# Kunvuthi/cobalt_smart_lender_ai

Hardware: AMD Instinct MI355X
Metric: rows/sec GBDT train on 10M-row LendingClub-shaped tabular; AUC parity (higher is better)
Workload: dtype fp32; 1 GPU; global_batch=10000000, rows_per_gpu=10000000, parallelism=dp1, n_features=20, trees=300, max_depth=7

## Files before the change

### cobalt_smart_lender_ai_amd/_native.py

```python
from __future__ import annotations

import ctypes
import os
import threading
from pathlib import Path

import torch

from . import build as _build
from .config import knob

_lock = threading.Lock()
_lib: ctypes.CDLL | None = None
_err: str | None = None

c_void_p = ctypes.c_void_p
c_int = ctypes.c_int
c_int64 = ctypes.c_int64
c_double = ctypes.c_double
c_float = ctypes.c_float
c_char_p = ctypes.c_char_p


class NativeUnavailable(RuntimeError):
    pass


_SIGS: dict[str, tuple] = {
    "cobalt_gbdt_create": (c_int, [c_void_p, ctypes.POINTER(c_void_p)]),
    "cobalt_heap_to_trees": (ctypes.c_int64, [c_void_p, c_int, c_int] + [c_void_p] * 10),
    "cobalt_gbdt_set_data": (c_int, [c_void_p] * 9),
    "cobalt_gbdt_grow": (c_int, [c_void_p, c_int, c_int, c_void_p]),
    "cobalt_gbdt_fetch_trees": (c_int, [c_void_p, c_int, c_int, c_void_p, c_void_p]),
    "cobalt_gbdt_max_nodes": (c_int, [c_void_p]),
    "cobalt_gbdt_set_start": (c_int, [c_void_p, c_int]),
    "cobalt_gbdt_set_binary_labels": (c_int, [c_void_p, c_float, c_void_p]),
    "cobalt_gbdt_set_monotone": (c_int, [c_void_p, c_void_p, c_int]),
    "cobalt_gbdt_set_interaction": (c_int, [c_void_p, c_void_p, c_int, c_int]),
    "cobalt_gbdt_destroy": (c_int, [c_void_p]),
    "cobalt_gbdt_reuse": (c_int, [c_void_p, c_void_p]),
    "cobalt_gbdt_grow_sampled": (c_int, [c_void_p, c_int, c_void_p]),
    "cobalt_gbdt_set_rows": (c_int, [c_void_p, c_int64]),
    "cobalt_gbdt_error": (c_int, [c_void_p]),
    "cobalt_gbdt_ox_init": (c_int, [c_void_p, c_int64, c_void_p, c_void_p, c_void_p]),
    "cobalt_gbdt_ox_begin": (c_int, [c_void_p, c_int, c_void_p]),
    "cobalt_gbdt_ox_page": (c_int, [c_void_p, c_void_p, c_int, c_int64, c_int64, c_int, c_int, c_void_p]),
    "cobalt_gbdt_ox_level": (c_int, [c_void_p, c_int, c_int, c_void_p]),
    "cobalt_gbdt_ox_end": (c_int, [c_void_p, c_int, c_void_p]),
    "cobalt_gbdt_set_fault": (c_int, [c_void_p, c_int]),
    "cobalt_gbdt_tree_ptr": (c_void_p, [c_void_p, c_int]),
    "cobalt_ooc_page": (c_int, [c_void_p, c_int, c_int64, c_int64, c_int, c_void_p, c_int, c_void_p, c_void_p, c_void_p,
                                ctypes.c_uint64, c_int64, ctypes.c_double, ctypes.c_double, ctypes.c_double,
                                c_void_p, c_void_p, c_int64, c_void_p, c_void_p, c_void_p]),
    "cobalt_ooc_bins": (c_int, []),
    "cobalt_gbdt_plan": (c_int, [c_void_p, c_void_p]),
# ... 118 lines not shown
```

### cobalt_smart_lender_ai_amd/config.py

```python
from __future__ import annotations

import dataclasses
import os
from dataclasses import dataclass, field
from pathlib import Path
from typing import Any

BUCKET_NAME = "cobalt-lending-ai-data-lake"
RAW_DATA_KEY_FULL = "dataset/1-raw/LendingClubFullData2007-2020Q3"
CLEAN_DATA_KEY_FULL = "dataset/2-intermediate/full_dataset_cleaned_01.csv"
RAW_DATA_KEY_SAMPLE = "dataset/1-raw/100kSampleData"
CLEAN_DATA_KEY_SAMPLE = "dataset/2-intermediate/sample_100k_cleaned.csv"
CLEAN_DATA_KEY_TREE = "dataset/2-intermediate/full_dataset_cleaned_02_tree.csv"
CLEAN_DATA_KEY_NN = "dataset/2-intermediate/full_dataset_cleaned_02_nn.csv"
MODEL_OUTPUT_PATH = "models/xgboost/"
BEST_MODEL_FILENAME = "xgb_model_tree.pkl"
FEATURES_FILENAME = "selected_features_tree.txt"
METRICS_JSON = "metrics.json"
S3_MODEL_KEY = "models/xgboost/xgb_model_tree.pkl"

LEAKAGE_COLUMNS = [
    "total_rec_late_fee", "total_rec_prncp", "out_prncp", "last_pymnt_amnt", "last_pymnt_d", "funded_amnt_inv",
    "funded_amnt", "out_prncp_inv", "total_pymnt", "total_pymnt_inv", "last_pymnt_d_days",
    "last_credit_pull_d_days", "issue_d_days", "total_rec_int",
# ... 89 lines not shown
    return cls(**{k: v for k, v in data.items() if k in names})


@dataclass(frozen=True)
class Knob:
    default: str
    scope: str
    doc: str


KNOBS: dict[str, Knob] = {
    "COBALT_STAMPS": Knob("", "native", "file: in-kernel launch / probe timestamps of sampled trees (scripts/stamp_summary.py)"),
    "COBALT_HIST_ABLATE": Knob("0", "native", "timing-only ablations of the histogram / partition / root passes (wrong models)"),
    "COBALT_HIST_CHUNK": Knob("auto", "native", "rows per histogram work item at levels >= 1 (~n/1536, 1024..4096)"),
    "COBALT_HIST_CHUNK0": Knob("auto", "native", "rows per root histogram item when the root pass is not fused"),
    "COBALT_ROOT_CHUNK": Knob("auto", "native", "rows per item of the fused gradient + root-histogram pass (whole rounds of 2 blocks per CU)"),
    "COBALT_PART_CHUNK": Knob("auto", "native", "rows per partition item (4096 while a level fits one block per CU, else 8192; <= 8192)"),
    "COBALT_EVAL_FG": Knob("auto", "native", "features per split-evaluation group (0 = one block per node; 8 above 32 features)"),
    "COBALT_EVAL_PART": Knob("1", "native", "split evaluation fused into the partition pass while a level fits one block per CU (0 off, 2 forced)"),
    "COBALT_HIST_PAIR": Knob("1", "native", "lane-pair record gathers in the histogram levels (16 < F <= 24)"),
    "COBALT_MAX_COPY_SHIFT": Knob("4", "native", "log2 of the per-lane LDS histogram copies of a low-cardinality feature (0..6)"),
    "COBALT_WT": Knob("auto", "native", "write-through stores: bit 0 histogram slabs, bit 1 partition row ids, bit 2 the root pass's (g, h) (7 below 4M rows, else 5)"),
    "COBALT_MARGIN_IN_RECORD": Knob("1", "native", "binary labels, <= 20 features, >= 4M rows: the root pass keeps every row's margin in its 32-byte record (0 off, 2 at any row count)"),
    "COBALT_PART_POS": Knob("1", "native", "row partition in position-ordered blocks whose row-id loads need no plan (0: node-ordered items)"),
    "COBALT_BIN_SCALAR": Knob("", "native", "force the generic binning kernel for 32-byte records (tests)"),
    "COBALT_PRED_WALK": Knob("4", "native", "trees walked at once per predictor thread (2 / 4 / 8)"),
    "COBALT_IPC_FUSED": Knob("1", "native", "IPC exchange fused into the split evaluation (0: separate exchange kernel + fused eval/partition)"),
    "COBALT_DP_OWNER": Knob("1", "native", "node ownership on the three deepest levels over the fused IPC exchange"),
    "COBALT_EVAL_BLOCKS": Knob("1", "native", "over the fused IPC exchange: the fused evaluation + partition pass with one evaluator block per node (0: k_eval + k_partition)"),
    "COBALT_CU_BUDGET": Knob("", "native", "CUs of this rank's CU-masked stream (set by parallel/cumask.py)"),
    "COBALT_DP_TRANSPORT": Knob("auto", "python", "native communicator: auto (IPC within a node), ipc or rccl"),
    "COBALT_DIST_BACKEND": Knob("auto", "python", "torch.distributed backend override (gloo for ranks sharing one GPU)"),
    "COBALT_DIST_NATIVE": Knob("auto", "python", "create the trainer's native communicator with a gloo bootstrap (1)"),
    "COBALT_IPC_SLOT_MB": Knob("64", "python", "IPC send-slot capacity per rank"),
    "COBALT_IPC_TIMEOUT_S": Knob("120", "python", "in-kernel exchange deadline before the group fails on every rank"),
    "COBALT_IPC_CONNECT_TIMEOUT_S": Knob("30", "python", "deadline of the IPC connect self-test"),
    "COBALT_COLLECTIVE_TIMEOUT_S": Knob("1800", "python", "host watchdog deadline for one enqueued segment of trees"),
    "COBALT_SHARED_CU_MASK": Knob("auto", "python", "CU-masked streams for ranks sharing one GPU (default for 2-8 ranks)"),
    "COBALT_CU_MASK_LAYOUT": Knob("blocked", "python", "CU masks of ranks sharing one GPU: blocked (contiguous bits, every XCC covered) or interleaved"),
    "COBALT_TEST_PLACEMENT": Knob("0", "test", "parallel/dp_check.py: record the XCCs / CUs a rank's masked stream runs on"),
    "COBALT_BENCH_SHARED_DEVICE": Knob("0", "python", "bench.py: every rank on cuda:0 (the 1-GPU multi-rank rehearsal)"),
    "COBALT_LABEL_IN_RECORD": Knob("1", "python", "0/1 labels ride in the row records' padding (weights derived from them)"),
    "COBALT_TRAINER_CACHE": Knob("1", "python", "keep one trainer context per process for back-to-back fits of the same shapes"),
    "COBALT_SEARCH_STREAMS": Knob("4", "python", "HIP streams of the randomized search's concurrent fits"),
    "COBALT_PRED_TILE": Knob("2048", "python", "tree nodes per LDS tile of the GPU predictor"),
    "COBALT_SK_TIMING": Knob("0", "python", "per-stage times of the device quantile sketch to stderr"),
# ... 24 lines not shown
```

### cobalt_smart_lender_ai_amd/csrc/gbdt.hip

```cpp
#include "common.h"
#include "comm.h"
#include "ipc_device.h"
#include "knobs.h"
#include <math.h>
#include <string.h>
#include <stdlib.h>
#include <vector>
#include <algorithm>
#include <type_traits>

using namespace cobalt;

namespace {

enum NodeStatus : int32_t { kNone = 0, kActive = 1, kSplit = 2, kLeaf = 3 };

struct Node {
  int64_t G, H;
  int32_t start, count;
  int32_t status, build;
  int32_t feat, bin;
  int32_t default_left;
  float split_cond;
  float loss_chg, leaf_value;
// ... 118 lines not shown
  double eta, lambda_, alpha, gamma, mcw, subsample, gscale, hscale, ginv, hinv;
  uint64_t seed;
  uint64_t* stamps;
  int32_t seq;
  int64_t* hist_red;
  int64_t* zero_red;
  const IpcFusedView* ipcv;
  unsigned ipc_epoch;
  int32_t wt;
  int32_t ylab;
  float spw;
  int32_t lab31;
  int32_t mrec;
  int64_t* dig;
  int32_t dig_slot;
  int32_t dig_check;
  int32_t world;
  int32_t corrupt;
  unsigned* err_host;
  int32_t ep_chunk, ep_zero;
  int32_t own_level;
  uint64_t* dec;
  int32_t wide;
};


__device__ __forceinline__ uint32_t node_hash(int n, int status, int feat, int bin, int dl, float cond, int64_t G,
                                              int64_t H) {
  uint64_t x = ((uint64_t)(uint32_t)n << 32) ^ ((uint64_t)(uint32_t)status << 40) ^ ((uint64_t)(uint32_t)feat << 44) ^
               ((uint64_t)(uint32_t)(bin & 0x3FF) << 52) ^ ((uint64_t)(uint32_t)dl << 62) ^ __float_as_uint(cond);
  x ^= (uint64_t)G * 0x9E3779B97F4A7C15ull;
  x ^= ((uint64_t)H << 29) | ((uint64_t)H >> 35);
  x ^= x >> 33;
  x *= 0xff51afd7ed558ccdull;
  x ^= x >> 33;
  x *= 0xc4ceb9fe1a85ec53ull;
  x ^= x >> 33;
  return (uint32_t)x;
}

__device__ __forceinline__ void digest_check(const GbdtDev& d, int64_t sum) {
  const int64_t own = d.dig_check ? d.dig[d.dig_slot ^ 1] : 0;
  if (sum != (int64_t)d.world * own) __hip_atomic_store(d.err_host, 2u, __ATOMIC_RELAXED, __HIP_MEMORY_SCOPE_SYSTEM);
}

__global__ void k_dig_stage(int64_t* dig, int slot) {
// ... 221 lines not shown
        uint32_t m = s_meta[0];
        while (m & kMetaSplit) {
          const int f = m & 0xFFFF, q = f >> 2;
          const uint32_t word = q == 0 ? ra.x : q == 1 ? ra.y : q == 2 ? ra.z : q == 3 ? ra.w : q == 4 ? rb.x : rb.y;
          const uint32_t b = (word >> (8 * (f & 3))) & 0xffu;
          const bool left = meta_left(m, b);
          n = 2 * n + (left ? 1 : 2);
          m = s_meta[n];
        }
        mf += s_leaf[n];
      } else {
        mf += tree_leaf_T(d, i, s_meta, s_leaf);
      }
      d.margin[i] = mf;
    }
    const double mm = (double)mf;
    const double p = 1.0 / (1.0 + exp(-mm));
    const uint32_t lbit = rb.z & 0x80000000u;
    const float yf = d.ylab ? (d.lab31 ? (lbit ? 1.0f : 0.0f) : (float)(rb.y >> 24)) : d.label[i];
    const double y = (double)yf;
    const double w = d.ylab ? (double)(yf != 0.0f ? d.spw : 1.0f) : (double)d.weight[i];
    double g = (p - y) * w;
    double h = fmax(p * (1.0 - p), 1e-16) * w;
    if (d.subsample < 1.0) {
      const uint64_t hsh = splitmix64(tree_key ^ (uint64_t)(d.row_offset + i));
      if (!(uniform01(hsh) < d.subsample)) { g = 0.0; h = 0.0; }
    }
    int64_t gq, hq;
    quantize_gh(g, h, d.gscale, d.hscale, dkey, d.row_offset + i, gq, hq, d.wide != 0);
    if (rec32) {
      rb.z = (uint32_t)hq | (d.lab31 ? lbit : 0u);
      rb.w = (uint32_t)(int32_t)gq;
      rec[1] = rb;
    } else {
      *reinterpret_cast<uint64_t*>(d.bins + i * d.stride + d.goff) =
          ((uint64_t)(uint32_t)(int32_t)gq << 32) | (uint64_t)(uint32_t)hq;
    }
  }
}

__global__ __launch_bounds__(256) void k_put_label31(uint8_t* bins, const float* label, int64_t n) {
  for (int64_t i = (int64_t)blockIdx.x * blockDim.x + threadIdx.x; i < n; i += (int64_t)gridDim.x * blockDim.x)
    reinterpret_cast<uint32_t*>(bins + i * 32)[6] = label[i] != 0.0f ? 0x80000000u : 0u;
}
__global__ __launch_bounds__(256) void k_margin_in(uint8_t* bins, const float* margin, int64_t n) {
  for (int64_t i = (int64_t)blockIdx.x * blockDim.x + threadIdx.x; i < n; i += (int64_t)gridDim.x * blockDim.x)
    reinterpret_cast<float*>(bins + i * 32)[5] = margin[i];
}
__global__ __launch_bounds__(256) void k_margin_label_in(uint8_t* bins, const float* margin, const float* label,
                                                         int64_t n) {
  for (int64_t i = (int64_t)blockIdx.x * blockDim.x + threadIdx.x; i < n; i += (int64_t)gridDim.x * blockDim.x) {
    uint32_t* w = reinterpret_cast<uint32_t*>(bins + i * 32);
// ... 416 lines not shown
    init_tree_block(d);
    if (threadIdx.x == 0) d.counters[0] = gridDim.x;
  }
  for (int i = threadIdx.x; i < entries * kW; i += blockDim.x) s_hist[i] = 0ull;
  flush_meta_store(fmeta, ft, s_fo, s_fs);
  hist_meta_store(lraw, s_fm, kCs);
  __syncthreads();
  stamp_.probe(1);
  const int item = blockIdx.x;
  const int64_t begin = (int64_t)item * chunk, end = min(d.n, begin + chunk);
  if (threadIdx.x == 0) {
    WorkItem w;
    w.node = 0; w.slot = 0; w.begin = (int32_t)begin; w.end = (int32_t)end;
    d.items_h[item] = w;
  }
  const HistLanes hl = hist_lanes_finish(lraw, ft, s_fm, kCs);
  const uint64_t tree_key = tree_key_of(d.seed, tree);
  const uint64_t dkey = splitmix64(tree_key ^ kDitherSalt);
  int64_t tg = 0, th = 0;
  const int B = blockDim.x;
  for (int64_t i0 = begin + threadIdx.x; i0 < end; i0 += U * B) {
    uint4 ra[U], rb[U];
    float mf[U], yl[U], wt[U];
#pragma unroll
    for (int u = 0; u < U; ++u) {
      const int64_t i = i0 + (int64_t)u * B;
      const int64_t ii = i < end ? i : begin;
      const uint4* rec = reinterpret_cast<const uint4*>(d.bins + ii * 32);
      ra[u] = rec[0];
      rb[u] = rec[1];
      mf[u] = d.mrec ? 0.0f : d.margin[ii];
      yl[u] = 0.0f;
      wt[u] = 0.0f;
      if (!d.ylab) {
        yl[u] = d.label[ii];
        wt[u] = d.weight[ii];
      }
    }
    float lf[U];
    const bool walk = apply_tree >= 0 && d.ablate != 22;
    if (walk) walk_leaves<U>(s_walk, d.max_depth, ra, rb, lf);
#pragma unroll
    for (int u = 0; u < U; ++u) {
      const int64_t i = i0 + (int64_t)u * B;
      if (i >= end) continue;
      if (d.mrec) mf[u] = __int_as_float((int)rb[u].y);
      if (walk) {
        mf[u] += lf[u];
        if (!d.mrec) d.margin[i] = mf[u];
      }
      const double mm = (double)mf[u];
      const double p = d.ablate == 20 ? 0.5 + 0.01 * mm : 1.0 / (1.0 + exp(-mm));
      const uint32_t lbit = rb[u].z & 0x80000000u;
      if (d.ylab) {
        yl[u] = d.lab31 ? (lbit ? 1.0f : 0.0f) : (float)(rb[u].y >> 24);
        wt[u] = yl[u] != 0.0f ? d.spw : 1.0f;
      }
      const double y = (double)yl[u];
      const double w = (double)wt[u];
      double g = (p - y) * w;
      double h = fmax(p * (1.0 - p), 1e-16) * w;
      if (d.subsample < 1.0) {
        const uint64_t hsh = splitmix64(tree_key ^ (uint64_t)(d.row_offset + i));
        if (!(uniform01(hsh) < d.subsample)) { g = 0.0; h = 0.0; }
      }
      int64_t gq, hq;
      quantize_gh(g, h, d.gscale, d.hscale, dkey, d.row_offset + i, gq, hq, kWide);
      tg += gq;
      th += hq;
      rb[u].y = d.mrec ? (uint32_t)__float_as_int(mf[u]) : rb[u].y;
      rb[u].z = (uint32_t)hq | (d.lab31 ? lbit : 0u);
      rb[u].w = (uint32_t)(int32_t)gq;
      if (!d.mrec && (d.wt & 4))
        store_wt(reinterpret_cast<uint64_t*>(d.bins + i * 32) + 3, ((uint64_t)rb[u].w << 32) | rb[u].z, true);
      else
        reinterpret_cast<uint4*>(d.bins + i * 32)[1] = rb[u];
      if (d.ablate != 21) hist_add_rec32<FT4, kWide>(s_hist, hl, ra[u], rb[u]);
    }
  }
  __syncthreads();
  stamp_.probe(2);
  hist_flush<kWide>(d, s_hist, hl, item, 0, ft, tg, th, true, s_tot, s_fo, s_fs);
}

template <int U, int FT4, bool kWide = false>
__global__ __launch_bounds__(kWide ? 1024 : 512) void k_grad_hist(GbdtDev d, int tree, int apply_tree, int chunk) {
  grad_hist_body<U, FT4, kWide>(d, tree, apply_tree, chunk);
}


// ... 1598 lines not shown
  uint64_t eval_asg[4] = {~0ull, ~0ull, ~0ull, ~0ull};
  EvalSlots eval_slots{};
  std::vector<int32_t> hoff_h;
  int fit_first = 0;
  int fault_tree = -1;
  uint32_t dec_tag = 0;
  bool label_pending = false;
  bool mono_on = false;
  bool inter_on = false;
  ConsDev cons{};
  int32_t plan[7] = {0, -1, 0, 0, 0, 0, 0};
  unsigned* err_pinned = nullptr;
  const char* stamp_path = nullptr;
  int stamp_cap = 0;
  uint64_t* stamp_buf = nullptr;
  std::vector<const char*> stamp_names;
  int64_t ox_n = 0;
  uint16_t* ox_pos = nullptr;
  uint64_t* ox_gh = nullptr;
  int64_t* ox_slab = nullptr;
  float* ox_margin = nullptr;
  const float* ox_label = nullptr;
  const float* ox_weight = nullptr;
};

static int stamp_next(GbdtCtx* c, const char* name) {
  if (!c->stamp_path || !c->d.stamps) return 0;
  if ((int)c->stamp_names.size() >= c->stamp_cap) { c->d.stamps = nullptr; return 0; }
  c->stamp_names.push_back(name);
  return (int)c->stamp_names.size() - 1;
}
#define GLAUNCH(tag, ...)               \
  do {                                  \
    c->d.seq = stamp_next(c, tag);      \
    hipLaunchKernelGGL(__VA_ARGS__);    \
  } while (0)
#define CONS_EVAL(kGroups, ...)                                                                        \
  do {                                                                                                 \
    if (c->mono_on && c->inter_on) GLAUNCH("k_eval", (k_eval_mono<kGroups, true, true>), __VA_ARGS__); \
    else if (c->inter_on) GLAUNCH("k_eval", (k_eval_mono<kGroups, false, true>), __VA_ARGS__);         \
    else GLAUNCH("k_eval", (k_eval_mono<kGroups, true, false>), __VA_ARGS__);                          \
  } while (0)
#define CONS_FINISH(...)                                                                                     \
  do {                                                                                                       \
    if (c->mono_on && c->inter_on) GLAUNCH("k_eval_finish", (k_eval_finish_mono<true, true>), __VA_ARGS__);  \
    else if (c->inter_on) GLAUNCH("k_eval_finish", (k_eval_finish_mono<false, true>), __VA_ARGS__);          \
// ... 253 lines not shown
  }
  for (int k = 0; k < 4; ++k) {
    uint64_t w = 0;
    for (int j = 0; j < 8; ++j) w |= (uint64_t)slot[k * 8 + j] << (8 * j);
    out[k] = w;
  }
}

COBALT_API int cobalt_gbdt_set_data(void* h, uint8_t* bins, const uint8_t* binsT, const float* cuts,
                                    const int32_t* nbins, const float* label, const float* weight,
                                    float* margin, const uint8_t* fmask) {
  GbdtCtx* c = static_cast<GbdtCtx*>(h);
  c->d.bins = bins;
  c->d.binsT = binsT;
  c->d.cuts = cuts;
  c->d.nbins = nbins;
  c->d.label = label;
  c->d.weight = weight;
  c->d.ylab = 0;
  c->d.lab31 = 0;
  c->label_pending = false;
  c->d.margin = margin;
  c->d.fmask = fmask;
  const int F = c->d.F, ft = c->d.feat_tile, ntiles = ceil_div(F, ft);
  std::vector<int32_t> nb(F);
  CK(hipMemcpy(nb.data(), nbins, F * sizeof(int32_t), hipMemcpyDeviceToHost));
  std::vector<int2> lay(F);
  std::vector<int32_t> ent(ntiles, 0);
  const int max_sh = std::min(6, std::max(0, knob_int(Knob::MaxCopyShift, 4)));
  int max_ent = 0;
  for (int t = 0; t < ntiles; ++t) {
    int off = 0;
    for (int f = t * ft; f < std::min(F, (t + 1) * ft); ++f) {
      const int b = std::max(1, std::min(256, nb[f]));
      int sh = 0;
      while (sh < max_sh && ((b + 1) << (sh + 1)) <= kMaxBins) ++sh;
      lay[f] = make_int2((f - t * ft) * kMaxBins, sh | (b >= 256 ? 8 : 0));
      off += kMaxBins;
    }
    ent[t] = off;
    max_ent = std::max(max_ent, off);
  }
  CK(hipMemcpy(c->d.layout, lay.data(), F * sizeof(int2), hipMemcpyHostToDevice));
  std::vector<int32_t> hoff(F + 1, 0);
  for (int f = 0; f < F; ++f) hoff[f + 1] = hoff[f] + std::max(1, std::min(256, nb[f]));
  CK(hipMemcpy(c->d.hoff, hoff.data(), (F + 1) * sizeof(int32_t), hipMemcpyHostToDevice));
// ... 49 lines not shown
  GbdtDev& d = c->d;
  const int D = d.max_depth;
  const int grad_grid = std::min(ceil_div(d.n, 256), 256 * 16);
  const int ftiles = ceil_div(d.F, d.feat_tile);
  const size_t tree_lds = (size_t)c->max_nodes * 8;
  const size_t walk_lds = (size_t)c->max_nodes * kWalkNodeBytes;
  if (t0 != c->grown) return -11;
  if (int rc = stamp_begin(c, stream)) return rc;
  const bool dp = c->cfg.comm != nullptr;
  d.dp = dp ? 1 : 0;
  CobaltComm* const cc = static_cast<CobaltComm*>(c->cfg.comm);
  const bool ipc = dp && cc->kind == 2;
  d.hist_red = nullptr;
  if (ipc) {
    if (ipc_capacity(cc) < ((int64_t)c->pairs_max * d.slot_elems + 2) * (int64_t)sizeof(int64_t)) {
      comm_set_error("ipc: slot capacity below one level of histograms (raise COBALT_IPC_SLOT_MB)");
      return -14;
    }
    if (int rc = ipc_zero_send(cc, d.slot_elems * (int64_t)sizeof(int64_t), stream)) return rc;
  }
  const int ft4 = hist_ft4(d);
  const bool fuse_root = !sampled && ft4 > 0 && ftiles == 1 && (d.ablate == 0 || d.ablate >= 10);
  if (d.wide && sampled) return -15;
  static const int env_mrec = knob_int(Knob::MarginInRecord, 1);
  d.mrec = (env_mrec != 0 && d.lab31 && fuse_root && d.n > 0 && (env_mrec == 2 || d.n >= 4000000)) ? 1 : 0;
  {
    const dim3 g1(std::max(1, std::min(ceil_div(d.n, 256), 4096)));
    if (c->label_pending && d.mrec)
      hipLaunchKernelGGL(k_margin_label_in, g1, dim3(256), 0, stream, d.bins, d.margin, d.label, d.n);
    else if (c->label_pending)
      hipLaunchKernelGGL(k_put_label31, g1, dim3(256), 0, stream, d.bins, d.label, d.n);
    else if (d.mrec)
      hipLaunchKernelGGL(k_margin_in, g1, dim3(256), 0, stream, d.bins, d.margin, d.n);
    if (c->label_pending || d.mrec) CK_LAUNCH();
    c->label_pending = false;
  }
  static const int env_fg = knob_int(Knob::EvalFg, -1);
  int eval_fg = env_fg >= 0 ? env_fg : (d.F > 32 ? 8 : 0);
  if (eval_fg == 0 && d.F > 32) eval_fg = 8;
  if (eval_fg > 0) eval_fg = std::min(32, std::max(eval_fg, ceil_div(d.F, 64)));
  const int env_ipc_fused = knob_int(Knob::IpcFused, 1);
  int fused_cells = c->d.ncells;
  if (eval_fg > 0) {
    fused_cells = 0;
    for (int f0 = 0; f0 < d.F; f0 += eval_fg)
      fused_cells = std::max(fused_cells, c->hoff_h[std::min(d.F, f0 + eval_fg)] - c->hoff_h[f0]);
  }
// ... 202 lines not shown
                       d.n);
    CK_LAUNCH();
    d.mrec = 0;
  }
  if (c->applied < c->grown) {
    GLAUNCH("k_apply_tree", k_apply_tree, dim3(std::max(grad_grid, 1)), dim3(256), tree_lds, stream, d, c->grown - 1);
    CK_LAUNCH();
    c->applied = c->grown;
  }
  if (dp && c->grown > t0) {
    const int ls = (c->grown - 1) & 1;
    hipLaunchKernelGGL(k_dig_stage, dim3(1), dim3(64), 0, stream, d.dig, ls);
    CK_LAUNCH();
    if (int rc = cobalt_comm_allreduce_sum_i64(c->cfg.comm, d.dig + 2, 1, stream)) return rc;
    hipLaunchKernelGGL(k_dig_cmp, dim3(1), dim3(64), 0, stream, d.dig, ls, d.world, d.err_host);
    CK_LAUNCH();
  }
  d.stamps = nullptr;
  return stamp_dump(c, stream);
}

COBALT_API int cobalt_gbdt_grow(void* h, int t0, int n_trees, hipStream_t stream) {
  return grow_impl(static_cast<GbdtCtx*>(h), t0, n_trees, stream, false);
}

constexpr int kOxSlab = 128;
constexpr int kOxFlushRows = 16384;
constexpr size_t kOxLdsBudget = 150 * 1024;

static int ox_group_slots(const GbdtDev& d) {
  return std::max<int>(1, (int)(kOxLdsBudget / ((size_t)(d.ncells + 1) * sizeof(uint64_t))));
}

__global__ __launch_bounds__(1024) void k_ox_page(GbdtDev d, const uint8_t* __restrict__ page, int ps, int64_t n,
                                                  int64_t r0, int mode, int tree, int apply, uint16_t* __restrict__ pos,
                                                  uint64_t* __restrict__ gh, int64_t* __restrict__ slab,
                                                  float* __restrict__ margin, const float* __restrict__ label,
                                                  const float* __restrict__ weight, int gslots) {
  extern __shared__ uint64_t s_h[];
  __shared__ uint32_t s_meta[256];
  __shared__ float s_leaf[256];
  __shared__ uint8_t s_build[256];
  __shared__ int s_hoff[kMaxFeatTile + 1];
  __shared__ int s_nb[kMaxFeatTile];
  const int F = d.F, nc = d.ncells, cells = nc + 1;
  const int g0 = blockIdx.y * gslots;
// ... 317 lines not shown
      (o.grad_bits > 17) != (cfg->grad_bits > 17))
    return 1;
  c->cfg = *cfg;
  GbdtDev& d = c->d;
  d.n = cfg->n_rows;
  d.row_offset = cfg->row_offset;
  d.eta = cfg->eta;
  d.lambda_ = cfg->lambda_;
  d.alpha = cfg->alpha;
  d.gamma = cfg->gamma;
  d.mcw = cfg->min_child_weight;
  d.subsample = cfg->subsample;
  d.gscale = cfg->gscale;
  d.hscale = cfg->hscale;
  d.ginv = 1.0 / cfg->gscale;
  d.hinv = 1.0 / cfg->hscale;
  d.seed = cfg->seed;
  c->grown = 0;
  c->applied = 0;
  c->fit_first = 0;
  c->fault_tree = -1;
  c->mono_on = false;
  c->inter_on = false;
  if (c->err_pinned) memset(c->err_pinned, 0, 64);
  return 0;
}

COBALT_API int cobalt_gbdt_destroy(void* h) {
  GbdtCtx* c = static_cast<GbdtCtx*>(h);
  if (!c) return 0;
  for (void* p : c->allocs) (void)hipFree(p);
  if (c->err_pinned) (void)hipHostFree(c->err_pinned);
  delete c;
  return 0;
}

template <int F4>
__global__ __launch_bounds__(256) void k_bin_rec32(const float* __restrict__ X, int64_t n,
                                                   const float* __restrict__ cuts, const int32_t* __restrict__ nbins,
                                                   uint8_t* __restrict__ bins, uint8_t* __restrict__ binsT,
                                                   int64_t ldt) {
  constexpr int F = 4 * F4;
  __shared__ float s_cuts[F * kMaxBins];
  __shared__ int s_nb[F];
  for (int i = threadIdx.x; i < F * kMaxBins; i += blockDim.x) s_cuts[i] = cuts[i];
  if (threadIdx.x < F) s_nb[threadIdx.x] = nbins[threadIdx.x];
// ... 96 lines not shown
```

### cobalt_smart_lender_ai_amd/models/gbdt.py

```python
from __future__ import annotations

import ctypes
import json
import logging
import math
import os
import time
from dataclasses import asdict, dataclass, field
from typing import Any, Sequence

import numpy as np
import torch

from . import gbdt_host, sketch
from .booster import Booster, dump_pickle_bytes, sigmoid32, trees_from_heap_nodes
from ..config import knob

log = logging.getLogger(__name__)

XGB_DEFAULTS = dict(n_estimators=100, max_depth=6, learning_rate=0.3, gamma=0.0, min_child_weight=1.0,
                    reg_lambda=1.0, reg_alpha=0.0, subsample=1.0, colsample_bytree=1.0, max_bin=256,
                    scale_pos_weight=1.0, random_state=0, base_score=None)


@dataclass
class GBDTParams:
    n_estimators: int = 100
    max_depth: int = 6
    learning_rate: float = 0.3
    gamma: float = 0.0
    min_child_weight: float = 1.0
    reg_lambda: float = 1.0
    reg_alpha: float = 0.0
    subsample: float = 1.0
    colsample_bytree: float = 1.0
    max_bin: int = 256
    scale_pos_weight: float = 1.0
    random_state: int = 0
    base_score: float | None = None
    sketch_rows: int | None = -1
    sketch_weight: str = "sample"
    sketch_mode: str = "sample"
    grad_bits: int = 17
    monotone_constraints: Any = None
    interaction_constraints: Any = None

    @classmethod
    def from_kwargs(cls, **kw) -> "GBDTParams":
        names = {f for f in cls.__dataclass_fields__}
        alias = {"eta": "learning_rate", "lambda": "reg_lambda", "alpha": "reg_alpha", "min_split_loss": "gamma",
                 "seed": "random_state"}
        out = {}
        for k, v in kw.items():
            k = alias.get(k, k)
            if k in names and v is not None:
                out[k] = v
        return cls(**out)


@dataclass
class FitReport:
    n_rows: int = 0
    n_rows_global: int = 0
    n_features: int = 0
    n_trees: int = 0
    device: str = "cpu"
    world: int = 1
    t_sketch: float = 0.0
# ... 343 lines not shown
    return out


def _refuse_interaction(params: "GBDTParams", what: str) -> None:
    if any(len(g) for g in _inter_plain(getattr(params, "interaction_constraints", None))):
        raise ValueError(f"interaction_constraints is not supported {what}")


def subset_interaction(groups: list[list[int]] | None, feats) -> list[list[int]] | None:
    if groups is None:
        return None
    pos = {int(f): i for i, f in enumerate(np.asarray(feats).reshape(-1).tolist())}
    out = [sorted(pos[f] for f in g if f in pos) for g in groups]
    return [g for g in out if g] or None


def interaction_words(groups: list[list[int]], n_features: int) -> np.ndarray:
    w = np.zeros(int(n_features), dtype=np.uint64)
    for k, g in enumerate(groups):
        w[np.asarray(g, dtype=np.int64)] |= np.uint64(1) << np.uint64(k)
    return w


def check_grad_bits(grad_bits: int, n_features: int, device_type: str) -> None:
    if grad_bits not in gbdt_host.GRAD_BITS:
        raise ValueError(f"grad_bits must be one of {gbdt_host.GRAD_BITS}")
    if grad_bits > 17 and device_type == "cuda" and n_features > 24:
        raise ValueError(f"grad_bits={grad_bits} on the GPU supports <= 24 features (32-byte row records); "
                         f"got {n_features}: use grad_bits=17")


def check_gpu_shape(max_depth: int, n_rows: int) -> None:
    if not 1 <= max_depth <= 10:
        raise ValueError(f"the GPU trainer supports max_depth 1-10 (got {max_depth}); use the host trainer "
                         "(device='cpu') for deeper trees")
    if n_rows >= (1 << 31) - 1:
        raise ValueError(f"{n_rows} rows exceed one GPU fit's int32 row ids: shard them over ranks "
                         "(data parallel) or stream them (models.external.train_external)")


class EvalMonitor:

    def __init__(self, evals, eval_metric=None, early_stopping_rounds: int | None = None, device=None,
                 n_features: int | None = None, verbose: bool = False):
        from .booster import check_eval_inputs

# ... 276 lines not shown

        margin = (init_margin.to(dev, torch.float32).clone().contiguous() if init_margin is not None
                  else torch.full((N,), base_margin, dtype=torch.float32, device=dev))
        comm = dist.native_comm if dist is not None else None
        if world > 1 and comm is None:
            raise RuntimeError("data-parallel GPU training needs the native RCCL communicator")
        tr = gbdt_ops.GpuGbdtTrainer(n_rows=N, n_feat=F, max_depth=hp.max_depth, max_trees=T, eta=hp.eta,
                                     reg_lambda=hp.reg_lambda, reg_alpha=hp.reg_alpha, gamma=hp.gamma,
                                     min_child_weight=hp.min_child_weight, subsample=hp.subsample,
                                     gscale=gscale, hscale=hscale, base_margin=base_margin,
                                     seed=hp.seed, row_offset=bd.row_offset, world_size=world, comm=comm,
                                     grad_bits=grad_bits)
        fm = torch.as_tensor(fmask_np, device=dev).contiguous()
        tr.set_data(bd.records, bd.binsT, bd.cuts.contiguous(), bd.nbins.to(torch.int32).contiguous(),
                    yt.contiguous(), wt, margin, fm)
        if (sample_weight is None and knob("COBALT_LABEL_IN_RECORD", "1") != "0"
                and bd.records.shape[1] == 32 and F <= 23
                and (labels_binary if labels_binary is not None else bool(((yt == 0) | (yt == 1)).all()))):
            tr.set_binary_labels(float(np.float32(spw)))
        if mono is not None:
            tr.set_monotone(mono)
        if inter is not None:
            tr.set_interaction(interaction_words(inter, F), len(inter))
        tp = rep.mark("trainer_setup", tp, dev)
        completed = False
        try:
            if T0:
                tr.set_start(T0)
            if world > 1:
                cr = int(knob("COBALT_FAULT_CORRUPT_RANK", "-1") or -1)
                if cr == dist.rank:
                    tr.set_fault(int(knob("COBALT_FAULT_CORRUPT_TREE", "1") or 1))
            head = None
            if checkpoint is None and not early and T - T0 >= 64 and _own_device(world):
                tail = min(32, (T - T0) // 4)
                head = T - tail
                tr.grow(T0, head - T0)
                ev = torch.cuda.Event()
                ev.record()
                tr.grow(head, T - head)
                rep.extra["plan"] = tr.plan()
                if world > 1:
                    _watch_segment(dist, dev, T0, head, tr, ev)
                else:
                    ev.synchronize()
                trees_so_far.extend(trees_from_heap_nodes(tr.fetch(T0, head - T0, _side_stream(dev)), hp.max_depth))
            for s0 in ([head] if head is not None else range(T0, T, seg)):
                s1 = min(T, s0 + seg)
                if head is None:
                    tr.grow(s0, s1 - s0)
                    rep.extra["plan"] = tr.plan()
                if world > 1:
                    _watch_segment(dist, dev, s0, s1, tr)
                tp = rep.mark("grow", tp, dev)
                seg_nodes = tr.fetch(s0, s1 - s0)
                if world > 1 and tr.replica_error():
                    raise ReplicaDivergence(f"data-parallel replicas diverged before tree {s1} (rank {dist.rank}): "
                                            "the ranks' split decisions differ (in-flight digest check)")
                tp = rep.mark("fetch", tp, dev)
                segment_done(seg_nodes, s1)
                tp = rep.mark("convert", tp, dev)
                if early_stop(s0):
                    break
            completed = True
        finally:
            tr.close(park=completed)
        tp = rep.mark("close", tp, dev)
        rep.extra["margin"] = margin
    else:
        cuts_np = bd.cuts.cpu().numpy()
        nb_np = bd.nbins.cpu().numpy()
        margin_np = (init_margin.cpu().numpy().astype(np.float32).copy() if init_margin is not None
                     else np.full(N, np.float32(base_margin), dtype=np.float32))
        y_np = yt.cpu().numpy()
        w_np = wt.cpu().numpy()
        allreduce = None
        if world > 1:
            def allreduce(a: np.ndarray) -> np.ndarray:
                t = torch.from_numpy(np.ascontiguousarray(a))
                dist.allreduce(t, "sum")
                return t.numpy()
        for s0 in range(T0, T, seg):
            s1 = min(T, s0 + seg)
            recs = []
            for t in range(s0, s1):
                gq, hq = gbdt_host.gradients_host(margin_np, y_np, w_np, hp, t, bd.row_offset)
# ... 367 lines not shown
```

### cobalt_smart_lender_ai_amd/ops/gbdt_ops.py

```python
from __future__ import annotations

import atexit
import os
import threading

import ctypes

import numpy as np
import torch

from .. import _native
from ..models.booster import NODE_DTYPE
from ..config import knob


class GbdtConfig(ctypes.Structure):
    _fields_ = [
        ("n_rows", ctypes.c_int64),
        ("row_offset", ctypes.c_int64),
        ("n_feat", ctypes.c_int32),
        ("row_stride", ctypes.c_int32),
        ("max_depth", ctypes.c_int32),
        ("max_trees", ctypes.c_int32),
        ("chunk", ctypes.c_int32),
# ... 177 lines not shown
        fn(self.h, out)
        return {"ipc_fused": bool(out[0]), "own_level": int(out[1]), "wide_gradients": bool(out[2]),
                "fused_eval_resident_blocks": int(out[3]),
                "eval_part_levels": [lv for lv in range(16) if (out[4] >> lv) & 1],
                "eval_block_levels": [lv for lv in range(16) if (out[5] >> lv) & 1],
                "eval_block_overflow_levels": [lv for lv in range(16) if (out[6] >> lv) & 1]}

    def replica_error(self) -> int:
        fn = getattr(self.lib, "cobalt_gbdt_error", None)
        return int(fn(self.h)) if (self.h and fn is not None) else 0

    def set_fault(self, tree: int) -> None:
        _native.check(self.lib.cobalt_gbdt_set_fault(self.h, int(tree)), "cobalt_gbdt_set_fault")

    def set_start(self, t0: int) -> None:
        _native.check(self.lib.cobalt_gbdt_set_start(self.h, t0), "cobalt_gbdt_set_start")

    def grow(self, t0: int, n_trees: int) -> None:
        rc = self.lib.cobalt_gbdt_grow(self.h, t0, n_trees, _native.stream_handle())
        if rc != 0 and self.cfg.comm:
            raise RuntimeError(f"cobalt_gbdt_grow failed ({rc}): {self.lib.cobalt_comm_last_error().decode()}")
        _native.check(rc, "cobalt_gbdt_grow")

    def set_rows(self, n: int) -> None:
        _native.check(self.lib.cobalt_gbdt_set_rows(self.h, int(n)), "cobalt_gbdt_set_rows")

    def grow_sampled(self, t: int) -> None:
        _native.check(self.lib.cobalt_gbdt_grow_sampled(self.h, t, _native.stream_handle()), "cobalt_gbdt_grow_sampled")

    def tree_ptr(self, t: int) -> int:
        return int(self.lib.cobalt_gbdt_tree_ptr(self.h, t))

    def fetch(self, t0: int, n: int, stream: torch.cuda.Stream | None = None) -> np.ndarray:
        out = np.zeros((n, self.max_nodes), dtype=NODE_DTYPE)
        rc = self.lib.cobalt_gbdt_fetch_trees(self.h, t0, n, out.ctypes.data, _native.stream_handle(stream))
        _native.check(rc, "cobalt_gbdt_fetch_trees")
        return out

    def close(self, park: bool = True) -> None:
        h = getattr(self, "h", None)
        if not h:
            return
        self.h = None
        self._keep = []
        if park and _cache_on() and getattr(self, "_key", None) is not None:
            with _PARKED_LOCK:
# ... 14 lines not shown
```

Before: 45.28 million rows/s.

## Regroup training rows by leaf after scheduled trees to improve locality

Adds a native counting-sort pass that walks a chosen tree, keys each row by its leaf, and permutes the 32-byte records, the transposed bins, margins, labels, weights and an original-index array into double-buffered copies. Later trees then read rows that sit together by leaf, which is meant to make partition and histogram memory access more contiguous. Sampling and quantization hashes use the original row index, so results stay deterministic. A final unpermute scatters margins back. The cost is extra device memory for two full copies and a sort pass at each scheduled tree. The native side refuses the reorder when margin-in-record is on, which is the default at this row count, so the Python side may fall back without reordering.

```diff
diff --git a/cobalt_smart_lender_ai_amd/_native.py b/cobalt_smart_lender_ai_amd/_native.py
--- a/cobalt_smart_lender_ai_amd/_native.py
+++ b/cobalt_smart_lender_ai_amd/_native.py
@@ -31,6 +31,8 @@
     "cobalt_heap_to_trees": (ctypes.c_int64, [c_void_p, c_int, c_int] + [c_void_p] * 10),
     "cobalt_gbdt_set_data": (c_int, [c_void_p] * 9),
     "cobalt_gbdt_grow": (c_int, [c_void_p, c_int, c_int, c_void_p]),
+    "cobalt_gbdt_reorder": (c_int, [c_void_p, c_int, c_void_p]),
+    "cobalt_gbdt_unpermute": (c_int, [c_void_p, c_void_p]),
     "cobalt_gbdt_fetch_trees": (c_int, [c_void_p, c_int, c_int, c_void_p, c_void_p]),
     "cobalt_gbdt_max_nodes": (c_int, [c_void_p]),
     "cobalt_gbdt_set_start": (c_int, [c_void_p, c_int]),
diff --git a/cobalt_smart_lender_ai_amd/config.py b/cobalt_smart_lender_ai_amd/config.py
--- a/cobalt_smart_lender_ai_amd/config.py
+++ b/cobalt_smart_lender_ai_amd/config.py
@@ -135,6 +135,7 @@
     "COBALT_MAX_COPY_SHIFT": Knob("4", "native", "log2 of the per-lane LDS histogram copies of a low-cardinality feature (0..6)"),
     "COBALT_WT": Knob("auto", "native", "write-through stores: bit 0 histogram slabs, bit 1 partition row ids, bit 2 the root pass's (g, h) (7 below 4M rows, else 5)"),
     "COBALT_MARGIN_IN_RECORD": Knob("1", "native", "binary labels, <= 20 features, >= 4M rows: the root pass keeps every row's margin in its 32-byte record (0 off, 2 at any row count)"),
+    "COBALT_ROW_REORDER": Knob("auto", "python", "trees after which the GPU trainer regroups the rows by leaf: '0,8,32', 'every:16', 'off' (auto: models/gbdt.py ROW_REORDER_AUTO by row count)"),
     "COBALT_PART_POS": Knob("1", "native", "row partition in position-ordered blocks whose row-id loads need no plan (0: node-ordered items)"),
     "COBALT_BIN_SCALAR": Knob("", "native", "force the generic binning kernel for 32-byte records (tests)"),
     "COBALT_PRED_WALK": Knob("4", "native", "trees walked at once per predictor thread (2 / 4 / 8)"),
diff --git a/cobalt_smart_lender_ai_amd/csrc/gbdt.hip b/cobalt_smart_lender_ai_amd/csrc/gbdt.hip
--- a/cobalt_smart_lender_ai_amd/csrc/gbdt.hip
+++ b/cobalt_smart_lender_ai_amd/csrc/gbdt.hip
@@ -164,6 +164,7 @@
   int32_t own_level;
   uint64_t* dec;
   int32_t wide;
+  const int32_t* orig;
 };
 
 
@@ -431,12 +432,13 @@
     const double w = d.ylab ? (double)(yf != 0.0f ? d.spw : 1.0f) : (double)d.weight[i];
     double g = (p - y) * w;
     double h = fmax(p * (1.0 - p), 1e-16) * w;
+    const int64_t gi = d.row_offset + (d.orig ? (int64_t)d.orig[i] : i);
     if (d.subsample < 1.0) {
-      const uint64_t hsh = splitmix64(tree_key ^ (uint64_t)(d.row_offset + i));
+      const uint64_t hsh = splitmix64(tree_key ^ (uint64_t)gi);
       if (!(uniform01(hsh) < d.subsample)) { g = 0.0; h = 0.0; }
     }
     int64_t gq, hq;
-    quantize_gh(g, h, d.gscale, d.hscale, dkey, d.row_offset + i, gq, hq, d.wide != 0);
+    quantize_gh(g, h, d.gscale, d.hscale, dkey, gi, gq, hq, d.wide != 0);
     if (rec32) {
       rb.z = (uint32_t)hq | (d.lab31 ? lbit : 0u);
       rb.w = (uint32_t)(int32_t)gq;
@@ -899,6 +901,7 @@
   for (int64_t i0 = begin + threadIdx.x; i0 < end; i0 += U * B) {
     uint4 ra[U], rb[U];
     float mf[U], yl[U], wt[U];
+    int32_t og[U];
 #pragma unroll
     for (int u = 0; u < U; ++u) {
       const int64_t i = i0 + (int64_t)u * B;
@@ -907,6 +910,7 @@
       ra[u] = rec[0];
       rb[u] = rec[1];
       mf[u] = d.mrec ? 0.0f : d.margin[ii];
+      og[u] = d.orig ? d.orig[ii] : (int32_t)i;
       yl[u] = 0.0f;
       wt[u] = 0.0f;
       if (!d.ylab) {
@@ -937,12 +941,13 @@
       const double w = (double)wt[u];
       double g = (p - y) * w;
       double h = fmax(p * (1.0 - p), 1e-16) * w;
+      const int64_t gi = d.row_offset + (int64_t)og[u];
       if (d.subsample < 1.0) {
-        const uint64_t hsh = splitmix64(tree_key ^ (uint64_t)(d.row_offset + i));
+        const uint64_t hsh = splitmix64(tree_key ^ (uint64_t)gi);
         if (!(uniform01(hsh) < d.subsample)) { g = 0.0; h = 0.0; }
       }
       int64_t gq, hq;
-      quantize_gh(g, h, d.gscale, d.hscale, dkey, d.row_offset + i, gq, hq, kWide);
+      quantize_gh(g, h, d.gscale, d.hscale, dkey, gi, gq, hq, kWide);
       tg += gq;
       th += hq;
       rb[u].y = d.mrec ? (uint32_t)__float_as_int(mf[u]) : rb[u].y;
@@ -2587,6 +2592,18 @@
   float* ox_margin = nullptr;
   const float* ox_label = nullptr;
   const float* ox_weight = nullptr;
+  uint8_t* ro_rec[2] = {nullptr, nullptr};
+  uint8_t* ro_T[2] = {nullptr, nullptr};
+  float* ro_margin[2] = {nullptr, nullptr};
+  float* ro_label[2] = {nullptr, nullptr};
+  float* ro_weight[2] = {nullptr, nullptr};
+  int32_t* ro_orig[2] = {nullptr, nullptr};
+  int32_t* ro_src = nullptr;
+  uint16_t* ro_key = nullptr;
+  int32_t* ro_cnt = nullptr;
+  int ro_cur = -1;
+  int ro_done = 0;
+  GbdtDev ro_user{};
 };
 
 static int stamp_next(GbdtCtx* c, const char* name) {
@@ -2886,6 +2903,9 @@
   c->label_pending = false;
   c->d.margin = margin;
   c->d.fmask = fmask;
+  c->d.orig = nullptr;
+  c->ro_cur = -1;
+  c->ro_done = 0;
   const int F = c->d.F, ft = c->d.feat_tile, ntiles = ceil_div(F, ft);
   std::vector<int32_t> nb(F);
   CK(hipMemcpy(nb.data(), nbins, F * sizeof(int32_t), hipMemcpyDeviceToHost));
@@ -2981,7 +3001,7 @@
   const int ft4 = hist_ft4(d);
   const bool fuse_root = !sampled && ft4 > 0 && ftiles == 1 && (d.ablate == 0 || d.ablate >= 10);
   if (d.wide && sampled) return -15;
-  static const int env_mrec = knob_int(Knob::MarginInRecord, 1);
+  const int env_mrec = knob_int(Knob::MarginInRecord, 1);
   d.mrec = (env_mrec != 0 && d.lab31 && fuse_root && d.n > 0 && (env_mrec == 2 || d.n >= 4000000)) ? 1 : 0;
   {
     const dim3 g1(std::max(1, std::min(ceil_div(d.n, 256), 4096)));
@@ -3230,6 +3250,220 @@
 
 COBALT_API int cobalt_gbdt_grow(void* h, int t0, int n_trees, hipStream_t stream) {
   return grow_impl(static_cast<GbdtCtx*>(h), t0, n_trees, stream, false);
+}
+
+constexpr int kRoChunk = 2048;
+constexpr int kRoWaves = 4;
+
+__global__ __launch_bounds__(256) void k_reorder_key(GbdtDev d, int tree, uint16_t* __restrict__ key) {
+  extern __shared__ uint32_t s_tree[];
+  uint32_t* s_meta = s_tree;
+  float* s_leaf = reinterpret_cast<float*>(s_tree + d.max_nodes);
+  stage_tree(d, d.trees + (int64_t)tree * d.max_nodes, s_meta, s_leaf);
+  __syncthreads();
+  for (int64_t i = (int64_t)blockIdx.x * blockDim.x + threadIdx.x; i < d.n; i += (int64_t)gridDim.x * blockDim.x) {
+    const uint4* rec = reinterpret_cast<const uint4*>(d.bins + i * 32);
+    const uint4 ra = rec[0], rb = rec[1];
+    int n = 0, level = 0;
+    uint32_t m = s_meta[0];
+    while ((m & kMetaSplit) && level < d.max_depth) {
+      const int f = m & 0xFFFF, q = f >> 2;
+      const uint32_t word = q == 0 ? ra.x : q == 1 ? ra.y : q == 2 ? ra.z : q == 3 ? ra.w : q == 4 ? rb.x : rb.y;
+      const uint32_t b = (word >> (8 * (f & 3))) & 0xffu;
+      n = 2 * n + (meta_left(m, b) ? 1 : 2);
+      ++level;
+      m = s_meta[n];
+    }
+    key[i] = (uint16_t)(((n + 1) << (d.max_depth - level)) - (1 << d.max_depth));
+  }
+}
+
+__global__ __launch_bounds__(kRoWaves * 64) void k_reorder_count(const uint16_t* __restrict__ key, int64_t n, int nk,
+                                                                 int nchunks, int32_t* __restrict__ cnt) {
+  extern __shared__ int32_t s_ro[];
+  const int w = threadIdx.x >> 6, lane = threadIdx.x & 63;
+  const int chunk = blockIdx.x * kRoWaves + w;
+  int32_t* my = s_ro + w * nk;
+  for (int k = lane; k < nk; k += 64) my[k] = 0;
+  __syncthreads();
+  for (int it = 0; it < kRoChunk / 64; ++it) {
+    const int64_t i = (int64_t)chunk * kRoChunk + it * 64 + lane;
+    if (chunk < nchunks && i < n) atomicAdd(&my[min((int)key[i], nk - 1)], 1);
+  }
+  __syncthreads();
+  if (chunk < nchunks)
+    for (int k = lane; k < nk; k += 64) cnt[(int64_t)k * nchunks + chunk] = my[k];
+}
+
+__global__ __launch_bounds__(1024) void k_reorder_scan(int32_t* __restrict__ a, int total) {
+  __shared__ int32_t s_w[16];
+  const int tid = threadIdx.x, w = tid >> 6, lane = tid & 63;
+  int32_t carry = 0;
+  for (int base = 0; base < total; base += 4096) {
+    const int idx = base + tid * 4;
+    int32_t v[4];
+#pragma unroll
+    for (int j = 0; j < 4; ++j) v[j] = idx + j < total ? a[idx + j] : 0;
+    const int32_t s = v[0] + v[1] + v[2] + v[3];
+    int32_t inc = s;
+#pragma unroll
+    for (int o = 1; o < 64; o <<= 1) {
+      const int32_t up = __shfl_up(inc, o, 64);
+      if (lane >= o) inc += up;
+    }
+    if (lane == 63) s_w[w] = inc;
+    __syncthreads();
+    int32_t before = 0, all = 0;
+#pragma unroll
+    for (int k = 0; k < 16; ++k) {
+      const int32_t t = s_w[k];
+      before += k < w ? t : 0;
+      all += t;
+    }
+    int32_t run = carry + before + inc - s;
+#pragma unroll
+    for (int j = 0; j < 4; ++j) {
+      if (idx + j < total) a[idx + j] = run;
+      run += v[j];
+    }
+    carry += all;
+    __syncthreads();
+  }
+}
+
+__global__ __launch_bounds__(kRoWaves * 64) void k_reorder_scatter(const uint16_t* __restrict__ key, int64_t n, int nk,
+                                                                   int nchunks, const int32_t* __restrict__ off,
+                                                                   int32_t* __restrict__ src) {
+  extern __shared__ int32_t s_ro[];
+  const int w = threadIdx.x >> 6, lane = threadIdx.x & 63;
+  const int chunk = blockIdx.x * kRoWaves + w;
+  int32_t* my = s_ro + w * nk;
+  if (chunk < nchunks)
+    for (int k = lane; k < nk; k += 64) my[k] = off[(int64_t)k * nchunks + chunk];
+  __syncthreads();
+  for (int it = 0; it < kRoChunk / 64; ++it) {
+    const int64_t i = (int64_t)chunk * kRoChunk + it * 64 + lane;
+    const bool valid = chunk < nchunks && i < n;
+    const int k = valid ? min((int)key[i], nk - 1) : -1;
+    int rank = 0, same = 0;
+    bool leader = false;
+    uint64_t rem = __ballot(valid);
+    while (rem) {
+      const int l = __ffsll((unsigned long long)rem) - 1;
+      const int k0 = __shfl(k, l, 64);
+      const uint64_t mk = __ballot(valid && k == k0);
+      if (valid && k == k0) {
+        rank = __popcll(mk & ((1ull << lane) - 1ull));
+        same = __popcll(mk);
+        leader = lane == l;
+      }
+      rem &= ~mk;
+    }
+    const int32_t first = valid ? my[k] : 0;
+    __syncthreads();
+    if (valid && (int64_t)first + rank < n) src[first + rank] = (int32_t)i;
+    if (leader) my[k] = first + same;
+    __syncthreads();
+  }
+}
+
+__global__ __launch_bounds__(256) void k_reorder_apply(GbdtDev d, const int32_t* __restrict__ src, uint8_t* __restrict__ rec_o,
+                                                       uint8_t* __restrict__ T_o, float* __restrict__ margin_o,
+                                                       float* __restrict__ label_o, float* __restrict__ weight_o,
+                                                       int32_t* __restrict__ orig_o) {
+  for (int64_t p = (int64_t)blockIdx.x * blockDim.x + threadIdx.x; p < d.n; p += (int64_t)gridDim.x * blockDim.x) {
+    const int64_t s = min((int64_t)(uint32_t)src[p], d.n - 1);
+    const uint4* rec = reinterpret_cast<const uint4*>(d.bins + s * 32);
+    const uint4 ra = rec[0], rb = rec[1];
+    uint4* out = reinterpret_cast<uint4*>(rec_o + p * 32);
+    out[0] = ra;
+    out[1] = rb;
+    margin_o[p] = d.margin[s];
+    if (!d.ylab) {
+      label_o[p] = d.label[s];
+      weight_o[p] = d.weight[s];
+    }
+    orig_o[p] = d.orig ? d.orig[s] : (int32_t)s;
+    const uint32_t wd[6] = {ra.x, ra.y, ra.z, ra.w, rb.x, rb.y};
+#pragma unroll
+    for (int f = 0; f < 24; ++f)
+      if (f < d.F) T_o[(int64_t)f * d.ldt + p] = (uint8_t)(wd[f >> 2] >> (8 * (f & 3)));
+  }
+}
+
+__global__ __launch_bounds__(256) void k_reorder_margin_out(const float* __restrict__ margin, const int32_t* __restrict__ orig,
+                                                            float* __restrict__ out, int64_t n) {
+  for (int64_t p = (int64_t)blockIdx.x * blockDim.x + threadIdx.x; p < n; p += (int64_t)gridDim.x * blockDim.x) {
+    const int64_t o = orig[p];
+    if (o >= 0 && o < n) out[o] = margin[p];
+  }
+}
+
+COBALT_API int cobalt_gbdt_reorder(void* h, int tree, hipStream_t stream) {
+  GbdtCtx* c = static_cast<GbdtCtx*>(h);
+  GbdtDev& d = c->d;
+  if (tree < 0 || tree >= c->grown || c->applied != c->grown) return -11;
+  if (hist_ft4(d) == 0 || d.wide || c->cfg.comm || d.n != d.ldt || d.n < 1 || d.mrec) return 1;
+  const int nk = 1 << d.max_depth;
+  const int nchunks = ceil_div(d.n, kRoChunk);
+  const int64_t total = (int64_t)nk * nchunks;
+  if (total > (1 << 24)) return 1;
+  const int64_t N = c->cfg.n_rows;
+  if (!c->ro_src) {
+    int rc = 0;
+    for (int k = 0; k < 2; ++k) {
+      if ((rc = dev_alloc(c, (void**)&c->ro_rec[k], (size_t)N * 32))) return rc;
+      if ((rc = dev_alloc(c, (void**)&c->ro_T[k], (size_t)N * d.F))) return rc;
+      if ((rc = dev_alloc(c, (void**)&c->ro_margin[k], (size_t)N * sizeof(float)))) return rc;
+      if ((rc = dev_alloc(c, (void**)&c->ro_label[k], (size_t)N * sizeof(float)))) return rc;
+      if ((rc = dev_alloc(c, (void**)&c->ro_weight[k], (size_t)N * sizeof(float)))) return rc;
+      if ((rc = dev_alloc(c, (void**)&c->ro_orig[k], (size_t)N * sizeof(int32_t)))) return rc;
+    }
+    if ((rc = dev_alloc(c, (void**)&c->ro_key, (size_t)N * sizeof(uint16_t)))) return rc;
+    if ((rc = dev_alloc(c, (void**)&c->ro_cnt, (size_t)nk * ceil_div(N, kRoChunk) * sizeof(int32_t)))) return rc;
+    if ((rc = dev_alloc(c, (void**)&c->ro_src, (size_t)N * sizeof(int32_t)))) return rc;
+  }
+  if (c->ro_cur < 0) c->ro_user = d;
+  const int nxt = c->ro_cur < 0 ? 0 : c->ro_cur ^ 1;
+  const dim3 g1(std::max(1, std::min(ceil_div(d.n, 256), 4096)));
+  const dim3 gs(ceil_div(nchunks, kRoWaves));
+  const size_t sort_lds = (size_t)kRoWaves * nk * sizeof(int32_t);
+  hipLaunchKernelGGL(k_reorder_key, g1, dim3(256), (size_t)c->max_nodes * 8, stream, d, tree, c->ro_key);
+  hipLaunchKernelGGL(k_reorder_count, gs, dim3(kRoWaves * 64), sort_lds, stream, c->ro_key, d.n, nk, nchunks, c->ro_cnt);
+  hipLaunchKernelGGL(k_reorder_scan, dim3(1), dim3(1024), 0, stream, c->ro_cnt, (int)total);
+  hipLaunchKernelGGL(k_reorder_scatter, gs, dim3(kRoWaves * 64), sort_lds, stream, c->ro_key, d.n, nk, nchunks, c->ro_cnt,
+                     c->ro_src);
+  hipLaunchKernelGGL(k_reorder_apply, g1, dim3(256), 0, stream, d, c->ro_src, c->ro_rec[nxt], c->ro_T[nxt],
+                     c->ro_margin[nxt], c->ro_label[nxt], c->ro_weight[nxt], c->ro_orig[nxt]);
+  CK_LAUNCH();
+  d.bins = c->ro_rec[nxt];
+  d.binsT = c->ro_T[nxt];
+  d.margin = c->ro_margin[nxt];
+  if (!d.ylab) {
+    d.label = c->ro_label[nxt];
+    d.weight = c->ro_weight[nxt];
+  }
+  d.orig = c->ro_orig[nxt];
+  c->ro_cur = nxt;
+  ++c->ro_done;
+  return 0;
+}
+
+COBALT_API int cobalt_gbdt_unpermute(void* h, hipStream_t stream) {
+  GbdtCtx* c = static_cast<GbdtCtx*>(h);
+  GbdtDev& d = c->d;
+  if (c->ro_cur < 0) return 0;
+  hipLaunchKernelGGL(k_reorder_margin_out, dim3(std::max(1, std::min(ceil_div(d.n, 256), 4096))), dim3(256), 0, stream,
+                     d.margin, d.orig, c->ro_user.margin, d.n);
+  CK_LAUNCH();
+  d.bins = c->ro_user.bins;
+  d.binsT = c->ro_user.binsT;
+  d.margin = c->ro_user.margin;
+  d.label = c->ro_user.label;
+  d.weight = c->ro_user.weight;
+  d.orig = nullptr;
+  c->ro_cur = -1;
+  return 0;
 }
 
 constexpr int kOxSlab = 128;
@@ -3593,6 +3827,9 @@
   c->fault_tree = -1;
   c->mono_on = false;
   c->inter_on = false;
+  d.orig = nullptr;
+  c->ro_cur = -1;
+  c->ro_done = 0;
   if (c->err_pinned) memset(c->err_pinned, 0, 64);
   return 0;
 }
diff --git a/cobalt_smart_lender_ai_amd/models/gbdt.py b/cobalt_smart_lender_ai_amd/models/gbdt.py
--- a/cobalt_smart_lender_ai_amd/models/gbdt.py
+++ b/cobalt_smart_lender_ai_amd/models/gbdt.py
@@ -44,6 +44,7 @@
     grad_bits: int = 17
     monotone_constraints: Any = None
     interaction_constraints: Any = None
+    row_reorder: Any = None
 
     @classmethod
     def from_kwargs(cls, **kw) -> "GBDTParams":
@@ -433,6 +434,30 @@
     return w
 
 
+ROW_REORDER_AUTO: list[tuple[int, str]] = [(1_000_000, "0"), (8_000_000, "0,8,32,128")]
+
+
+def resolve_row_reorder(spec, n_trees: int, n_rows: int) -> list[int]:
+    if spec is None:
+        spec = knob("COBALT_ROW_REORDER", "auto")
+    if isinstance(spec, str):
+        s = spec.strip().lower()
+        if s == "auto":
+            s = "off"
+            for min_rows, sched in ROW_REORDER_AUTO:
+                if n_rows >= min_rows:
+                    s = sched
+        if s in ("", "off"):
+            return []
+        spec = int(s[6:]) if s.startswith("every:") else [int(t) for t in s.split(",") if t.strip()]
+    if isinstance(spec, (int, np.integer)):
+        spec = range(0, n_trees, int(spec)) if int(spec) > 0 else []
+    out = sorted({int(t) for t in spec})
+    if out and out[0] < 0:
+        raise ValueError("row_reorder: tree indices must be >= 0")
+    return [t for t in out if t < n_trees - 1]
+
+
 def check_grad_bits(grad_bits: int, n_features: int, device_type: str) -> None:
     if grad_bits not in gbdt_host.GRAD_BITS:
         raise ValueError(f"grad_bits must be one of {gbdt_host.GRAD_BITS}")
@@ -755,6 +780,26 @@
             tr.set_monotone(mono)
         if inter is not None:
             tr.set_interaction(interaction_words(inter, F), len(inter))
+        ro_sched = resolve_row_reorder(params.row_reorder, T, N)
+        ro_off = ("data parallel" if world > 1 else "init_booster" if init_booster is not None or T0
+                  else "checkpointing" if checkpoint is not None
+                  else "generic records" if bd.records.shape[1] != 32 or F > 24
+                  else "wide gradients" if grad_bits != 17 else None) if ro_sched else "no schedule"
+        ro_done: list[int] = []
+
+        def grow(a: int, n: int) -> None:
+            nonlocal ro_off
+            b = a + n
+            for r in ([] if ro_off else [r for r in ro_sched if a <= r < b]):
+                tr.grow(a, r + 1 - a)
+                a = r + 1
+                if tr.reorder(r):
+                    ro_done.append(r)
+                else:
+                    ro_off = "not supported for this fit by the native trainer"
+                    break
+            if b > a:
+                tr.grow(a, b - a)
         tp = rep.mark("trainer_setup", tp, dev)
         completed = False
         try:
@@ -768,10 +813,10 @@
             if checkpoint is None and not early and T - T0 >= 64 and _own_device(world):
                 tail = min(32, (T - T0) // 4)
                 head = T - tail
-                tr.grow(T0, head - T0)
+                grow(T0, head - T0)
                 ev = torch.cuda.Event()
                 ev.record()
-                tr.grow(head, T - head)
+                grow(head, T - head)
                 rep.extra["plan"] = tr.plan()
                 if world > 1:
                     _watch_segment(dist, dev, T0, head, tr, ev)
@@ -781,7 +826,7 @@
             for s0 in ([head] if head is not None else range(T0, T, seg)):
                 s1 = min(T, s0 + seg)
                 if head is None:
-                    tr.grow(s0, s1 - s0)
+                    grow(s0, s1 - s0)
                     rep.extra["plan"] = tr.plan()
                 if world > 1:
                     _watch_segment(dist, dev, s0, s1, tr)
@@ -795,6 +840,8 @@
                 tp = rep.mark("convert", tp, dev)
                 if early_stop(s0):
                     break
+            tr.unpermute()
+            rep.extra["row_reorder"] = {"trees": ro_done, "off": ro_off}
             completed = True
         finally:
             tr.close(park=completed)
diff --git a/cobalt_smart_lender_ai_amd/ops/gbdt_ops.py b/cobalt_smart_lender_ai_amd/ops/gbdt_ops.py
--- a/cobalt_smart_lender_ai_amd/ops/gbdt_ops.py
+++ b/cobalt_smart_lender_ai_amd/ops/gbdt_ops.py
@@ -223,6 +223,16 @@
             raise RuntimeError(f"cobalt_gbdt_grow failed ({rc}): {self.lib.cobalt_comm_last_error().decode()}")
         _native.check(rc, "cobalt_gbdt_grow")
 
+    def reorder(self, tree: int) -> bool:
+        rc = self.lib.cobalt_gbdt_reorder(self.h, int(tree), _native.stream_handle())
+        if rc == 1:
+            return False
+        _native.check(rc, "cobalt_gbdt_reorder")
+        return True
+
+    def unpermute(self) -> None:
+        _native.check(self.lib.cobalt_gbdt_unpermute(self.h, _native.stream_handle()), "cobalt_gbdt_unpermute")
+
     def set_rows(self, n: int) -> None:
         _native.check(self.lib.cobalt_gbdt_set_rows(self.h, int(n)), "cobalt_gbdt_set_rows")
 
```

Result: faster. 48.67 million rows/s (median of 6 runs) (+7.5%).
